# sreeramkannan/Shannon

Measured on AMD Instinct MI355X. Metric: reads/sec k-mer->graph->path-decompose, 2x100bp k=25, higher is better.
Workload: dtype u64

## Files before the change

shannon_amd/csrc/extend.hip:

```cpp
#include "common.h"
#include <cstring>
#include <vector>
#include <time.h>
#include <cstdio>
#include <cstdlib>
#include <algorithm>

#define EBLK 256
#define WBLK 64
#define UNCLAIMED 0xFFFFFFFFu
#define NONE32 0xFFFFFFFFu
#define UNCLAIMED64 0xFFFFFFFFFFFFFFFFULL
#define NOHINT_WORD 0xFFFFFFFFu
#define LONG_WALK 8
#define MEMO_MIN 1
#define PROMOTE_STEPS 16
typedef unsigned long long u64;
#define CLAIM(rank, pos) (((u64)(rank) << 32) | (u64)(uint32_t)(pos))
#define RANK(c) ((uint32_t)((c) >> 32))
#define POS(c) ((uint32_t)(c))

struct Adj4 { int32_t v[4]; };
struct __attribute__((aligned(64))) Rec {
  Adj4 R;
// ... 1171 lines not shown
  if (isd && lg) long_list[bl + ol + __popcll(lm & below)] = (uint32_t)r;
  if (isd && !lg) short_list[bs + os + __popcll(sm & below)] = (uint32_t)r;
}

__global__ void ext_memo_plan_kernel(uint8_t* __restrict__ ran, uint8_t* __restrict__ dirty,
                                     const uint32_t* __restrict__ nr, const uint32_t* __restrict__ nl, const uint32_t* __restrict__ order,
                                     uint32_t frozen, uint32_t limit, uint64_t* __restrict__ moff, uint32_t* __restrict__ mR,
                                     uint32_t* __restrict__ mL, uint8_t* __restrict__ mvalid, uint8_t* __restrict__ fill,
                                     uint32_t* __restrict__ pool, unsigned long long* __restrict__ cursor, uint64_t pool_cap, uint32_t memo_min,
                                     uint32_t* __restrict__ log_head = nullptr) {
  uint64_t r = (uint64_t)blockIdx.x * blockDim.x + threadIdx.x + frozen;
  if (r >= limit) return;
  const uint8_t did_run = dirty[r];
  ran[r] = did_run;
  dirty[r] = 0;
  if (log_head && did_run && memo_min != 0xFFFFFFFFu) log_head[r] = (nr[r] != UNCLAIMED && nr[r] + nl[r] == 0) ? NONE32 : LOG_LOST;
  uint8_t f = 0;
  if (did_run && nr[r] != UNCLAIMED) {
    const uint32_t R = nr[r], L = nl[r];
    if (R + L >= memo_min) {
      const uint64_t cap = (uint64_t)R + L + 5;
      const unsigned long long off = atomicAdd(cursor, (unsigned long long)cap);
      if (off + cap + 64 <= pool_cap) {
        pool[off] = MEMO_MARK; pool[off + 1] = R | MEMO_HI; pool[off + 2] = order[r];
        pool[off + 3 + R] = MEMO_MARK; pool[off + 4 + R + L] = MEMO_MARK;
        moff[r] = off; mR[r] = R; mL[r] = L; mvalid[r] = 2; f = 1;
      }
    }
  }
  if (did_run && !f && mvalid[r]) mvalid[r] = 1;
  fill[r] = f;
}

__global__ __launch_bounds__(64) void ext_release_memo_kernel(const uint32_t* __restrict__ long_list, uint64_t n_long, const uint32_t* __restrict__ short_list,
                                                              uint64_t n_short, const uint32_t* __restrict__ nr, const uint64_t* __restrict__ moff,
                                                              const uint32_t* __restrict__ mR, const uint32_t* __restrict__ mL, const uint32_t* __restrict__ pool,
                                                              u64* claim, uint8_t* __restrict__ chunk, const uint8_t* __restrict__ mvalid = nullptr,
                                                              const uint32_t* __restrict__ order = nullptr, const uint32_t* __restrict__ logpool = nullptr,
                                                              const uint32_t* __restrict__ log_head = nullptr, const uint8_t* __restrict__ log_cnt = nullptr) {
  const uint64_t idx = blockIdx.x;
  if (idx >= n_long + n_short) return;
  const uint32_t r = idx < n_long ? long_list[idx] : short_list[idx - n_long];
  if (nr[r] == UNCLAIMED) return;
  if (mvalid && mvalid[r] != 2) {
    auto give_back = [&](uint32_t node) {
      const u64 c = __hip_atomic_load(&claim[node], __ATOMIC_RELAXED, __HIP_MEMORY_SCOPE_AGENT);
      if (RANK(c) == r && atomicCAS(&claim[node], c, UNCLAIMED64) == c && chunk) chunk[node >> CHUNK_SHIFT] = 1;
    };
    if (threadIdx.x == 0) give_back(order[r]);
    uint32_t ch = log_head[r], cnt = log_cnt[r];
    while (ch != NONE32 && ch != LOG_LOST) {
      const uint32_t* c = logpool + (uint64_t)ch * LOG_WORDS;
      if (threadIdx.x >= 1 && threadIdx.x <= cnt) give_back(c[threadIdx.x]);
      ch = c[0];
      cnt = LOG_PER;
    }
    return;
  }
  const uint64_t off = moff[r];
  const uint32_t R = mR[r], L = mL[r];
  for (uint32_t j = threadIdx.x; j <= R + L; j += 64) {
    const uint32_t node = pool[off + (j <= R ? 2 : 3) + j];
    if (node & 0x80000000u) continue;
    if (atomicCAS(&claim[node], CLAIM(r, j), UNCLAIMED64) == CLAIM(r, j) && chunk) chunk[node >> CHUNK_SHIFT] = 1;
  }
}
// ... 82 lines not shown
#undef MARK
  };
  if (!chunk) {
    for (uint64_t ch = wave; ch < n_groups; ch += n_waves) {
      const uint64_t y = (ch << 6) + lane;
      uint32_t a;
      if (y < n2 && mark_node(y, a)) mark_around(y, a);
    }
  } else {
    static_assert(CHUNK_SHIFT == 4, "four line flags per group of 64 k1-mers");
    const uint64_t n_super = (n_groups + 63) >> 6;
    for (uint64_t sg = wave; sg < n_super; sg += n_waves) {
      const uint64_t g = (sg << 6) + lane;
      const uint32_t fl = g < n_groups ? *(const uint32_t*)(chunk + g * 4) : 0u;
      unsigned long long todo = __ballot(fl != 0);
      while (todo) {
        const int j = __ffsll((long long)todo) - 1;
        todo &= todo - 1;
        const uint32_t flj = (uint32_t)__shfl((int)fl, j, 64);
        const uint64_t y = ((((sg << 6) + (uint64_t)j)) << 6) + lane;
        uint32_t a = 0;
        if (y < n2 && ((flj >> (8 * (lane >> 4))) & 0xFFu) && mark_node(y, a)) mark_around(y, a);
      }
    }
  }
  __shared__ unsigned long long blk_changed;
  if (threadIdx.x == 0) blk_changed = 0;
  __syncthreads();
  if (my_changed) atomicAdd(&blk_changed, (unsigned long long)my_changed);
  __syncthreads();
  if (threadIdx.x == 0 && blk_changed) atomicAdd(n_changed, blk_changed);
}

__global__ void ext_verify_kernel(const uint8_t* __restrict__ ran, uint8_t* __restrict__ robbed, uint64_t ns, uint8_t* __restrict__ dirty) {
  uint64_t r = (uint64_t)blockIdx.x * blockDim.x + threadIdx.x;
  if (r >= ns) return;
  if (robbed[r]) { robbed[r] = 0; if (ran[r]) dirty[r] = 1; }
}

__global__ void ext_seed_rank_kernel(const uint32_t* __restrict__ order, uint64_t ns, Rec* __restrict__ rec) {
  uint64_t r = (uint64_t)blockIdx.x * blockDim.x + threadIdx.x;
  if (r < ns) rec[order[r]].seed_rank = (uint32_t)r;
}

__global__ void ext_select_kernel(const uint32_t* __restrict__ ranks, uint64_t n_sel, int32_t* __restrict__ sel_of_rank,
                                  unsigned long long* __restrict__ n_twice) {
  uint64_t t = (uint64_t)blockIdx.x * blockDim.x + threadIdx.x;
  if (t >= n_sel) return;
  if (atomicCAS((int*)&sel_of_rank[ranks[t]], -1, (int)t) != -1) atomicAdd(n_twice, 1ULL);
}

__global__ void ext_emit_claims_kernel(const u64* __restrict__ claim, uint64_t n2, const int32_t* __restrict__ sel_of_rank, uint64_t ns,
                                       const uint32_t* __restrict__ nr_a, const uint32_t* __restrict__ nl_a,
                                       const uint64_t* __restrict__ tkeys, int k, const uint64_t* __restrict__ out_off,
                                       uint8_t* __restrict__ out_bases, unsigned long long* __restrict__ counters) {
  uint32_t n_wrote = 0, n_stray = 0;
  for (uint64_t y = (uint64_t)blockIdx.x * blockDim.x + threadIdx.x; y < n2; y += (uint64_t)gridDim.x * blockDim.x) {
    const u64 c = claim[y];
    const uint32_t r = RANK(c), pos = POS(c);
    if (r == UNCLAIMED || r >= ns) continue;
    const int32_t t = sel_of_rank[r];
    if (t < 0) continue;
    const uint32_t nr = nr_a[r], nl = nl_a[r];
    if (nr == UNCLAIMED || pos > nr + nl) { n_stray++; continue; }
    uint8_t* dst = out_bases + out_off[t];
    const uint64_t str = oriented_string(tkeys, (uint32_t)y, k);
    if (pos == 0) for (int j = 0; j < k; j++) dst[nl + j] = "ACGT"[(str >> (2 * (k - 1 - j))) & 3];
    else if (pos <= nr) dst[nl + k + (pos - 1)] = "ACGT"[str & 3];
    else dst[nl - 1 - (pos - nr - 1)] = "ACGT"[(str >> (2 * (k - 1))) & 3];
    n_wrote++;
// ... 539 lines not shown
  if (!e->has_dig) return shn_fail(SHN_ERR_ARG, "shn_ext_digests: the extension was not made with SHN_EXT_DIGEST=1");
  memcpy(out, e->dig, sizeof e->dig);
  return SHN_OK;
}

extern "C" int shn_extend(shn_ctx* ctx, const shn_table* t, uint32_t min_weight, int max_iterations, shn_ext** out) {
  return shn_extend_sharded(ctx, t, min_weight, max_iterations, 1, 0, out);
}

extern "C" int shn_extend_sharded(shn_ctx* ctx, const shn_table* t, uint32_t min_weight, int max_iterations, int world, int rank,
                                  shn_ext** out) {
  if (!ctx || !t || !out) return shn_fail(SHN_ERR_ARG, "shn_extend: NULL argument");
  if (world < 1 || world > 255 || rank < 0 || rank >= world) return shn_fail(SHN_ERR_ARG, "shn_extend_sharded: bad world/rank");
  if (2 * t->n >= 0x7FFFFFFFULL) return shn_fail(SHN_ERR_ARG, "shn_extend: table too large for 31-bit oriented ids");
  SHN_ENTER(ctx);
  shn_stage_begin(ctx);
  hipStream_t s = ctx->stream; shn_use_stream(s);
  if (world > 1 && t->n) {
    shn_table* sub = nullptr;
    int rcs;
    { TimerRegion treg(ctx, T_EXTEND); rcs = component_shard(ctx, t, world, rank, &sub); }
    if (rcs) return rcs;
    rcs = shn_extend_sharded(ctx, sub, min_weight, max_iterations, 1, 0, out);
    if (rcs) { shn_table_destroy(sub); return rcs; }
    (*out)->owned_table = sub;
    return SHN_OK;
  }
  TimerRegion treg(ctx, T_EXTEND);
  shn_ext* e = new shn_ext();
  memset(e, 0, sizeof(*e));
  e->ctx = ctx; e->device = ctx->device; e->k = t->k; e->n = t->n; e->min_weight = min_weight; e->table = t;
  uint64_t n = t->n;
  if (max_iterations <= 0) max_iterations = 100000;
#define TRYE(x) do { hipError_t _e = (x); if (_e != hipSuccess) { shn_ext_destroy(e); \
      return shn_fail(SHN_ERR_HIP, std::string(#x) + ": " + hipGetErrorString(_e)); } } while (0)
  TRYE(shn_dev_malloc(&e->d_weight, (n + 1) * 4));
  TRYE(shn_dev_malloc(&e->d_flags, n + 1));
  TRYE(shn_dev_malloc(&e->d_rec, (2 * n + 1) * sizeof(Rec)));
  const uint64_t claim_words = (2 * n + 4 + 31) & ~31ULL;
  { u64* both = nullptr;
    TRYE(shn_dev_malloc(&both, std::max<uint64_t>(2 * claim_words * 8, fine_dict_lines(t) * 128)));
    e->d_claim = both; e->d_claim2 = both + claim_words; }
  if (n) {
    TimerRegion t1(ctx, T_EXT_PREP);
    hipLaunchKernelGGL(ext_prepare_kernel, dim3((uint32_t)cdiv(n, 256)), dim3(256), 0, s, t->d_keys, t->d_counts, n, t->k,
                       t->canonical, e->d_weight, e->d_flags);
    {
      unsigned long long* lines = nullptr;
      uint64_t n_lines = 0;
      { int rca = build_fine_dict(ctx, t, e->d_flags, &lines, &n_lines, e->d_claim); if (rca) { shn_ext_destroy(e); return rca; } }
      static const bool rec_lds = getenv("SHN_REC_LDS") && getenv("SHN_REC_LDS")[0] == '1';
      if (t->layout == 1 && rec_lds && t->n_buckets / REC_G + 1 < 0x7FFFFFFFULL) {
        TimerRegion ta(ctx, T_EXT_ADJ);
        hipLaunchKernelGGL(ext_records_lds_kernel, dim3((uint32_t)cdiv(t->n_buckets, REC_G)), dim3(256), 0, s, shn_tab_idx(t), e->d_flags, e->d_weight,
                           (uint64_t)t->n_buckets, t->k, t->canonical, e->d_rec, (const unsigned long long*)lines,
                           getenv("SHN_REC_ABLATE") ? atoi(getenv("SHN_REC_ABLATE")) : 0);
      } else
      { TimerRegion ta(ctx, T_EXT_ADJ);
        hipLaunchKernelGGL(ext_records_kernel, dim3((uint32_t)std::min<uint64_t>(cdiv(n * 8, 256), 1u << 22)), dim3(256), 0, s, shn_tab_idx(t),
                           e->d_flags, e->d_weight, n, t->k, t->canonical, e->d_rec, (const unsigned long long*)lines, n_lines,
                           (getenv("SHN_XCD_MAP") && getenv("SHN_XCD_MAP")[0] == '1') ? 1 : 0); }
      (void)lines;
    }
    TRYE(hipGetLastError());
  }
  void *pk, *pv, *pk2, *pv2, *pc;
  int rc;
  if ((rc = shn_ws(ctx)[13].get(2048, &pc))) { shn_ext_destroy(e); return rc; }
  unsigned long long* d_cnt = (unsigned long long*)pc;
  TRYE(hipMemsetAsync(d_cnt, 0, 2048, s));
  const uint64_t n_sblk = cdiv(n, 1024);
  uint32_t* d_bcnt = nullptr; uint64_t* d_bbase = nullptr;
  struct SeedScratch { uint32_t** a; uint64_t** b; ~SeedScratch() { if (*a) shn_dev_free(*a); if (*b) shn_dev_free(*b); } } seed_scratch{&d_bcnt, &d_bbase};
  TRYE(shn_dev_malloc(&d_bcnt, (n_sblk + 1) * 4));
  TRYE(shn_dev_malloc(&d_bbase, (n_sblk + 2) * 8));
  if (n) hipLaunchKernelGGL(ext_seed_kernel, dim3((uint32_t)n_sblk), dim3(1024), 0, s, t->d_keys, e->d_weight, e->d_flags, n,
                            t->k, t->canonical, min_weight, d_bcnt, (const uint64_t*)nullptr, (uint64_t*)nullptr, (uint32_t*)nullptr);
  uint64_t ns = 0;
  if (n && (rc = shn_device_scan_u32(ctx, d_bcnt, n_sblk, d_bbase, &ns))) { shn_ext_destroy(e); return rc; }
  if ((rc = shn_ws(ctx)[9].get((ns + 2) * 8, &pk)) || (rc = shn_ws(ctx)[10].get((ns + 2) * 4, &pv)) ||
      (rc = shn_ws(ctx)[11].get((ns + 2) * 8, &pk2)) || (rc = shn_ws(ctx)[12].get((ns + 2) * 4, &pv2))) { shn_ext_destroy(e); return rc; }
  uint64_t* skeys = (uint64_t*)pk; uint32_t* svals = (uint32_t*)pv;
  if (n) hipLaunchKernelGGL(ext_seed_kernel, dim3((uint32_t)n_sblk), dim3(1024), 0, s, t->d_keys, e->d_weight, e->d_flags, n,
                            t->k, t->canonical, min_weight, d_bcnt, (const uint64_t*)d_bbase, skeys, svals);
  e->n_seeds = ns;
  {
    TimerRegion t2(ctx, T_EXT_SORT);
    if ((rc = shn_sort_pairs(ctx, skeys, svals, (uint64_t*)pk2, (uint32_t*)pv2, ns, 0, 2 * t->k))) { shn_ext_destroy(e); return rc; }
    if (ns) {
      hipLaunchKernelGGL(ext_weightkey_kernel, dim3((uint32_t)cdiv(ns, 256)), dim3(256), 0, s, svals, e->d_weight, ns, skeys);
      if ((rc = shn_sort_pairs(ctx, skeys, svals, (uint64_t*)pk2, (uint32_t*)pv2, ns, 0, 32))) { shn_ext_destroy(e); return rc; }
    }
  }
  TRYE(shn_dev_malloc(&e->d_order, (ns + 1) * 4));
  TRYE(shn_dev_malloc(&e->d_nr, (ns + 1) * 4));
  TRYE(shn_dev_malloc(&e->d_nl, (ns + 1) * 4));
  TRYE(shn_dev_malloc(&e->d_totw, (ns + 1) * 8));
  uint64_t pool_cap = std::min<uint64_t>(24 * n + (1ULL << 20), (1ULL << 30) - 1);
  if (getenv("SHN_EXT_POOL_WORDS")) pool_cap = std::max<uint64_t>(256, std::min<uint64_t>(pool_cap, strtoull(getenv("SHN_EXT_POOL_WORDS"), nullptr, 10)));
  TRYE(hipMemcpyAsync(e->d_order, svals, ns * 4, hipMemcpyDeviceToDevice, s));
  TRYE(hipMemsetAsync(e->d_nr, 0xFF, (ns + 1) * 4, s));
  TRYE(hipMemsetAsync(e->d_nl, 0, (ns + 1) * 4, s));
  TRYE(hipMemsetAsync(e->d_totw, 0, (ns + 1) * 8, s));
  TRYE(hipMemsetAsync(e->d_claim, 0xFF, (2 * n + 4) * 8, s));
  void *ppool, *pplan;
  if ((rc = shn_ws(ctx)[27].get(pool_cap * 4, &ppool)) ||
      (rc = shn_ws(ctx)[28].get((ns + 1) * (8 + 4 * 10 + 1 + 1 + 1 + 1 + 1 + 1 + 1) + 64, &pplan))) { shn_ext_destroy(e); return rc; }
  u64 *claim = e->d_claim, *snap = e->d_claim2;
  uint32_t* pool = (uint32_t*)ppool;
  uint64_t* moff = (uint64_t*)pplan;
  uint32_t* mcap = (uint32_t*)(moff + ns + 1);
  uint32_t* mR = mcap + ns + 1;
  uint32_t* mL = mR + ns + 1;
  uint32_t* long_list = mL + ns + 1;
  uint32_t* short_list = long_list + ns + 1;
  uint32_t* promo_list = short_list + ns + 1;
  uint32_t* res_cur = promo_list + ns + 1;
  uint32_t* res_info = res_cur + ns + 1;
  uint32_t* owned = res_info + ns + 1;
  uint32_t* log_head = owned + ns + 1;
  uint8_t* mvalid = (uint8_t*)(log_head + ns + 1);
  uint8_t* fill = mvalid + ns + 1;
  uint8_t* dirty = fill + ns + 1;
  uint8_t* ran = dirty + ns + 1;
  uint8_t* robbed = ran + ns + 1;
  uint8_t* settled = robbed + ns + 1;
  uint8_t* log_cnt = settled + ns + 1;
  TRYE(hipMemsetAsync(robbed, 0, 2 * (ns + 1), s));
  TRYE(hipMemsetAsync(log_head, 0xFE, (ns + 1) * 4, s));
  uint8_t* robsat = nullptr;
  struct RobsatFree { uint8_t** p; ~RobsatFree() { if (*p) shn_dev_free(*p); } } robsat_free{&robsat};
  if (getenv("SHN_EXT_XTIME")) { TRYE(shn_dev_malloc(&robsat, ns + 1)); TRYE(hipMemsetAsync(robsat, 0, ns + 1, s)); }
  TRYE(hipMemsetAsync(mvalid, 0, 2 * (ns + 1), s));
  TRYE(hipMemsetAsync(pool, 0xFF, pool_cap * 4, s));
  if (ns) hipLaunchKernelGGL(ext_seed_rank_kernel, dim3((uint32_t)cdiv(ns, 256)), dim3(256), 0, s, e->d_order, (uint64_t)ns, e->d_rec);
  const bool want_dig = getenv("SHN_EXT_DIGEST") && getenv("SHN_EXT_DIGEST")[0] == '1';
  if (want_dig) {
    int rd;
    if ((rd = ext_digest(ctx, e, 0, t->d_keys, n * 8, 1)) || (rd = ext_digest(ctx, e, 1, t->d_counts, n * 4, 2)) ||
        (rd = ext_digest(ctx, e, 2, t->d_bucket_off, (t->n_buckets + 1) * 8, 3)) || (rd = ext_digest(ctx, e, 3, e->d_weight, n * 4, 4)) ||
        (rd = ext_digest(ctx, e, 3, e->d_flags, n & ~3ULL, 5)) || (rd = ext_digest(ctx, e, 4, e->d_rec, 2 * n * sizeof(Rec), 6)) ||
        (rd = ext_digest(ctx, e, 5, e->d_order, ns * 4, 7))) { shn_ext_destroy(e); return rd; }
  }
  hipStream_t aux = nullptr;
  hipEvent_t ev_fork = nullptr, ev_join = nullptr;
  TRYE(hipStreamCreateWithFlags(&aux, hipStreamNonBlocking));
  TRYE(hipEventCreateWithFlags(&ev_fork, hipEventDisableTiming));
  TRYE(hipEventCreateWithFlags(&ev_join, hipEventDisableTiming));
  static thread_local unsigned long long* plan = nullptr;
  if (!plan) TRYE(hipHostMalloc((void**)&plan, 64));
  int it = 0, repairs = 0;
  bool converged = ns == 0;
  uint8_t* chunk = nullptr;
  const uint64_t n_chunks = ((2 * n) >> CHUNK_SHIFT) + 16;
  TRYE(shn_dev_malloc(&chunk, n_chunks));
  struct ChunkFree { uint8_t* p; ~ChunkFree() { shn_dev_free(p); } } chunk_free{chunk};
  TRYE(hipMemsetAsync(chunk, 0, n_chunks, s));
  uint8_t* coarse = nullptr;
  TRYE(shn_dev_malloc(&coarse, (size_t)ns / 64 + 64));
  struct CoarseFree { uint8_t* p; ~CoarseFree() { shn_dev_free(p); } } coarse_free{coarse};
  bool snap_current = false;
  bool fresh_block = true;

  const uint32_t g2n = (uint32_t)cdiv(2 * n, 256);
  const bool many = ns >= (1ULL << 24);
  unsigned long long lim0 = std::max<unsigned long long>(ns / (many ? 8 : 32), 4096), grow = 4;
  if (getenv("SHN_EXT_LIMIT0")) lim0 = strtoull(getenv("SHN_EXT_LIMIT0"), nullptr, 10);
  if (getenv("SHN_EXT_GROW")) grow = strtoull(getenv("SHN_EXT_GROW"), nullptr, 10);
  const unsigned long long tail_div = getenv("SHN_EXT_TAIL") ? strtoull(getenv("SHN_EXT_TAIL"), nullptr, 10) : (many ? 0 : 8);
  uint32_t frozen = 0, limit = (uint32_t)std::min<unsigned long long>(ns, lim0);
  TRYE(hipMemsetAsync(dirty, 0, 2 * (ns + 1), s));
  TRYE(hipMemsetAsync(dirty, 1, limit, s));
  TRYE(hipMemsetAsync(owned, 0, (ns + 1) * 4, s));
  plan[6] = 64;
  TRYE(hipMemcpyAsync(d_cnt + 10, plan + 6, 8, hipMemcpyHostToDevice, s));
  auto tune = [](const char* name, uint32_t dflt) { const char* v = getenv(name); return v ? (uint32_t)strtoul(v, nullptr, 10) : dflt; };
  const int precise_marks = (int)tune("SHN_EXT_PRECISE", 1);
  const uint32_t long_walk = tune("SHN_EXT_LONG_WALK", LONG_WALK), memo_min = tune("SHN_EXT_MEMO_MIN", MEMO_MIN),
                 promote_steps = tune("SHN_EXT_PROMOTE", PROMOTE_STEPS);
  const unsigned long long bulk_min = getenv("SHN_EXT_BULK") ? strtoull(getenv("SHN_EXT_BULK"), nullptr, 10) : 262144ULL;
  const unsigned long long dense_min = getenv("SHN_EXT_DENSE") ? strtoull(getenv("SHN_EXT_DENSE"), nullptr, 10) : (4ULL << 20);
  const int seed_check = (int)tune("SHN_EXT_SEEDCHECK", 1);
  const int first_look = (int)tune("SHN_EXT_FIRST_LOOK", 0);
  const uint32_t bulk_promote = tune("SHN_EXT_PROMOTE_BULK", 0);
  const unsigned long long resume_waves = tune("SHN_EXT_RESUME_WAVES", 8192);
  const bool skip_idle_begin = tune("SHN_EXT_MEMO_RELEASE", 1) != 0;
  const unsigned long long memo_release_max = tune("SHN_EXT_MEMO_RELEASE_MAX", 65536);
  int n_begin_skipped = 0;
  const bool prepass = tune("SHN_EXT_PREPASS", 1) != 0;
  const uint32_t settle_hops = tune("SHN_EXT_SETTLE_HOPS", 0);
  const bool use_logs = tune("SHN_EXT_LOGS", 1) != 0 && bulk_promote == 0 && ns > 0;
  const unsigned long long targeted_max_steps = getenv("SHN_EXT_TARGETED_MAX") ? strtoull(getenv("SHN_EXT_TARGETED_MAX"), nullptr, 10) : (12ULL << 20);
  uint32_t* logpool = nullptr;
  struct LogFree { uint32_t** p; ~LogFree() { if (*p) shn_dev_free(*p); } } log_free{&logpool};
  uint64_t log_cap = use_logs ? std::min<uint64_t>(2 * n / 4 + (1u << 16), 0x7FFFFFF0ULL) : 0;
  if (use_logs && getenv("SHN_EXT_LOG_CHUNKS")) log_cap = std::max<uint64_t>(LOG_SLAB, std::min<uint64_t>(log_cap, strtoull(getenv("SHN_EXT_LOG_CHUNKS"), nullptr, 10)));
  if (use_logs) { TRYE(shn_dev_malloc(&logpool, log_cap * LOG_WORDS * 4)); TRYE(hipMemsetAsync(d_cnt + 26, 0, 8, s)); }
  const uint32_t fresh_split = std::max<uint32_t>(1, std::min<uint32_t>(16, tune("SHN_EXT_FRESH_SPLIT", 1)));
  const uint32_t fresh_split_min = tune("SHN_EXT_FRESH_SPLIT_MIN", 65536);
  unsigned long long expect_dirty = limit;
  while (!converged && it < max_iterations) {
    const bool bulk = bulk_min && expect_dirty >= bulk_min;
    const bool dense = bulk && expect_dirty >= dense_min;
    TRYE(hipMemsetAsync(d_cnt + 2, 0, 32, s));
    TRYE(hipMemsetAsync(d_cnt + 24, 0, 8, s));
    if (limit > frozen)
      hipLaunchKernelGGL(ext_plan_kernel, dim3((uint32_t)cdiv(limit - frozen, 1024)), dim3(1024), 0, s, e->d_nr, e->d_nl, (uint64_t)limit, frozen,
                         mvalid, mR, mL, dirty, long_list, short_list, d_cnt + 2, bulk ? 0xFFFFFFFFu : long_walk, coarse,
                         (fresh_block && frozen > 0 && prepass) ? (const u64*)claim : (const u64*)nullptr, e->d_order, e->d_totw,
                         (const Rec*)e->d_rec, fresh_block ? settle_hops : 0u, settled, d_cnt + 20, robsat, d_cnt + 21,
                         use_logs ? (const uint32_t*)log_head : (const uint32_t*)nullptr, d_cnt + 24);
    TRYE(hipMemcpyAsync(plan, d_cnt + 2, 32, hipMemcpyDeviceToHost, s));
    TRYE(hipMemcpyAsync(plan + 7, d_cnt + 24, 8, hipMemcpyDeviceToHost, s));
    TRYE(hipStreamSynchronize(s));
    expect_dirty = plan[3];
    if (plan[3] == 0) {
      if (limit >= ns) {
        TimerRegion ta(ctx, T_EXT_AUDIT);
        TRYE(hipMemsetAsync(owned, 0, (ns + 1) * 4, s));
        TRYE(hipMemsetAsync(d_cnt + 48, 0, 16, s));
        hipLaunchKernelGGL(ext_audit_nodes_kernel, dim3(std::min<uint32_t>(g2n, 4096u)), dim3(256), 0, s, claim, 2 * n, rows_R(e->d_rec),
                           rows_L(e->d_rec), words_weight(e->d_rec), e->d_order, e->d_nr, e->d_nl, (uint64_t)ns, owned, dirty, d_cnt + 48);
        hipLaunchKernelGGL(ext_audit_walks_kernel, dim3((uint32_t)cdiv(ns, 256)), dim3(256), 0, s, claim, e->d_order, e->d_nr, e->d_nl, (uint64_t)ns,
                           owned, dirty, d_cnt + 48);
        TRYE(hipMemcpyAsync(plan + 4, d_cnt + 48, 16, hipMemcpyDeviceToHost, s));
        TRYE(hipStreamSynchronize(s));
        if (plan[4] == 0 && plan[5] == 0) {
          converged = true;
          if (g_block_cb) g_block_cb(g_block_user, e, frozen, ns, 1);
          break;
        }
        if (g_block_cb) g_block_cb(g_block_user, e, 0, 0, -1);
        fprintf(stderr, "[shn_extend] fixpoint audit after %d rounds: %llu k1-mers / %llu walks disagree with the greedy rule; reopening all blocks\n",
                it, plan[4], plan[5]);
        if (++repairs > 16) break;
        fresh_block = false;
        frozen = 0;
        expect_dirty = plan[4] + plan[5];
        TRYE(hipMemsetAsync(ran, 0, ns + 1, s));
// ... 79 lines not shown
    if (plan[2]) {
      TimerRegion tk(ctx, fresh_block ? T_EXT_WALK_FRESH : T_EXT_WALK_THREAD);
      if (fresh_block) hipLaunchKernelGGL(ext_walk_kernel<true>, dim3((uint32_t)cdiv(plan[2], WBLK)), dim3(WBLK), 0, s, A, (uint64_t)plan[2], short_list, snap);
      else hipLaunchKernelGGL(ext_walk_kernel<false>, dim3((uint32_t)cdiv(plan[2], WBLK)), dim3(WBLK), 0, s, A, (uint64_t)plan[2], short_list, snap);
    }
    if (x_t0 > 0) {
      TRYE(hipStreamSynchronize(s)); timespec ts; clock_gettime(CLOCK_MONOTONIC, &ts);
      unsigned long long st = 0, lw = 0; TRYE(hipMemcpyAsync(&st, d_cnt + 1, 8, hipMemcpyDeviceToHost, s));
      if (A.dbg) { TRYE(hipMemcpyAsync(&lw, d_cnt + 44, 8, hipMemcpyDeviceToHost, s)); TRYE(hipMemsetAsync(d_cnt + 44, 0, 8, s)); }
      TRYE(hipStreamSynchronize(s));
      unsigned long long nrs[3] = {0, 0, 0}; TRYE(hipMemcpyAsync(nrs, d_cnt + 21, 24, hipMemcpyDeviceToHost, s)); TRYE(hipMemsetAsync(d_cnt + 21, 0, 24, s)); TRYE(hipStreamSynchronize(s));
      fprintf(stderr, "[shn_extend] XTIME round %d [%u,%u): of the claim holders without a memo %llu were robbed while they sat out; their walks: longest %llu steps, %llu steps in all\n", it + 1, frozen, limit, nrs[0], nrs[1], nrs[2]);
      fprintf(stderr, "[shn_extend] XTIME round %d: release %s (claims to give back by the records: %llu; bulk %d dense %d fresh %d snapshot current %d)\n", it + 1,
              was_fresh ? "none (a new block)" : memo_release_done ? "through memos / logs" : "the begin pass", plan[7], (int)bulk, (int)dense, (int)was_fresh, (int)snap_was_current);
      fprintf(stderr, "[shn_extend] XTIME round %d: %llu dirty walks, %llu of them hold claims without a current memo (rounds released through memos so far: %d); thread walker %llu walks, %.2f ms, steps so far %llu; longest walk %llu steps in %.2f ms (%.2f us per step)\n", it + 1, plan[3], plan[1], n_begin_skipped, plan[2],
              ts.tv_sec * 1e3 + ts.tv_nsec * 1e-6 - x_t0, st, lw >> 32, (double)(lw & 0xFFFFFFFFULL) * 1e-5, (lw >> 32) ? (double)(lw & 0xFFFFFFFFULL) * 1e-2 / (double)(lw >> 32) : 0.0);
    }
    if (plan[2] && bulk) {
      if (bulk_promote) {
        TimerRegion tk(ctx, T_EXT_WALK_THREAD);
        const uint32_t rgrid = (uint32_t)std::min<unsigned long long>(cdiv(plan[2], WBLK), resume_waves);
        if (was_fresh) hipLaunchKernelGGL(ext_walk_resume_kernel<true>, dim3(rgrid), dim3(WBLK), 0, s, A, promo_list, (const unsigned long long*)(d_cnt + 13), d_cnt + 14, snap);
        else hipLaunchKernelGGL(ext_walk_resume_kernel<false>, dim3(rgrid), dim3(WBLK), 0, s, A, promo_list, (const unsigned long long*)(d_cnt + 13), d_cnt + 14, snap);
      }
    } else if (plan[2]) {
      TimerRegion tk(ctx, T_EXT_WALK_WAVE);
      hipLaunchKernelGGL(ext_walk_long_kernel<true>, dim3((uint32_t)std::min<unsigned long long>(plan[2], 8192ULL)), dim3(64), 0, s, A, promo_list,
                         (uint64_t)ns, (const unsigned long long*)(d_cnt + 13));
    }
    if (plan[0]) TRYE(hipStreamWaitEvent(s, ev_join, 0));
    const bool skip_mark = fresh_block && bulk && precise_marks;
    fresh_block = false;
    if (dense) e->dense_rounds++;
    hipLaunchKernelGGL(ext_memo_plan_kernel, dim3((uint32_t)cdiv(limit - frozen, 256)), dim3(256), 0, s, ran, dirty, e->d_nr, e->d_nl, e->d_order, frozen, limit,
                       moff, mR, mL, mvalid, fill, pool, d_cnt + 10, pool_cap, bulk ? 0xFFFFFFFFu : memo_min, use_logs ? log_head : (uint32_t*)nullptr);
    if (skip_mark) { snap_current = false; if (!dense) TRYE(hipMemsetAsync(chunk, 0, n_chunks, s)); }
    else
    { TimerRegion tk(ctx, T_EXT_MARK);
      hipLaunchKernelGGL(ext_mark_kernel, dim3(std::min<uint32_t>(g2n, 4096u)), dim3(256), 0, s, claim, snap, 2 * n, e->d_rec,
                         dirty, ran, d_cnt + 6, frozen, limit, bulk ? (const uint8_t*)nullptr : (const uint8_t*)fill, moff, mR, pool, e->d_nr, e->d_nl, precise_marks,
                         dense ? (const uint8_t*)nullptr : chunk, robsat);
      if (!dense) TRYE(hipMemsetAsync(chunk, 0, n_chunks, s)); }
    hipLaunchKernelGGL(ext_verify_kernel, dim3((uint32_t)cdiv(ns, 256)), dim3(256), 0, s, ran, robbed, (uint64_t)ns, dirty);
    if (getenv("SHN_EXT_FAULT") && it + 1 == atoi(getenv("SHN_EXT_FAULT"))) TRYE(hipMemsetAsync(dirty, 0, ns + 1, s));
    if (getenv("SHN_EXT_ALLDIRTY")) { TRYE(hipMemsetAsync(dirty, 0, ns + 1, s)); TRYE(hipMemsetAsync(dirty + frozen, 1, limit - frozen, s)); }
    it++;

    if (getenv("SHN_DEBUG")) {
      unsigned long long chg = 0, cur = 0, mx[2] = {0, 0}, st_tr[2] = {0, 0};
      TRYE(hipMemcpyAsync(&st_tr[0], d_cnt + 1, 8, hipMemcpyDeviceToHost, s));
      TRYE(hipMemcpyAsync(&st_tr[1], d_cnt + 15, 8, hipMemcpyDeviceToHost, s));
      TRYE(hipMemcpyAsync(&chg, d_cnt + 6, 8, hipMemcpyDeviceToHost, s));
      TRYE(hipMemcpyAsync(&cur, d_cnt + 10, 8, hipMemcpyDeviceToHost, s));
      TRYE(hipMemcpyAsync(mx, d_cnt + 42, 16, hipMemcpyDeviceToHost, s));
      TRYE(hipMemsetAsync(d_cnt + 42, 0, 16, s));
      TRYE(hipStreamSynchronize(s));
      static double t_prev = 0;
      timespec ts; clock_gettime(CLOCK_MONOTONIC, &ts);
      double tn = ts.tv_sec * 1e3 + ts.tv_nsec * 1e-6;
      static unsigned long long st_prev[2] = {0, 0};
      if (it == 1) { st_prev[0] = st_prev[1] = 0; }
      fprintf(stderr, "[shn_extend] round %d [%u,%u): dirty=%llu long=%llu short=%llu changed_kmers=%llu pool=%.1f%% longest wavefront walk: %llu steps, most sequential: %llu (no hint %llu, owner without memo %llu, memo moved on %llu, followed %llu)  thread steps %llu in %llu wavefront trips (lanes busy %.3f)  %.2f ms\n", it, frozen, limit,
              plan[3], plan[0], plan[2], chg, 100.0 * (double)cur / (double)pool_cap, mx[1], mx[0] >> 48, (mx[0] >> 36) & 4095, (mx[0] >> 24) & 4095, (mx[0] >> 12) & 4095, mx[0] & 4095,
              st_tr[0] - st_prev[0], st_tr[1] - st_prev[1], (double)(st_tr[0] - st_prev[0]) / (64.0 * (double)std::max<unsigned long long>(1, st_tr[1] - st_prev[1])), it == 1 ? 0.0 : tn - t_prev);
      st_prev[0] = st_tr[0]; st_prev[1] = st_tr[1];
      t_prev = tn;
    }
  }
  hipStreamSynchronize(aux);
  hipStreamDestroy(aux);
  hipEventDestroy(ev_fork);
  hipEventDestroy(ev_join);
  if (converged && ns && getenv("SHN_EXT_AUDIT")) {
    WalkArgs A;
    memset(&A, 0, sizeof(A));
    A.order = e->d_order; A.adjR = rows_R(e->d_rec); A.adjL = rows_L(e->d_rec); A.weight = words_weight(e->d_rec);
    A.claim = claim; A.nr_out = e->d_nr; A.nl_out = e->d_nl; A.totw_out = e->d_totw;
    unsigned long long au[2] = {0, ~0ULL};
    plan[4] = 0; plan[5] = ~0ULL;
    TRYE(hipMemcpyAsync(d_cnt + 48, plan + 4, 16, hipMemcpyHostToDevice, s));
    hipLaunchKernelGGL(ext_audit_kernel, dim3((uint32_t)cdiv(ns, 64)), dim3(64), 0, s, A, (uint64_t)ns, d_cnt + 48);
    TRYE(hipMemcpyAsync(plan + 4, d_cnt + 48, 16, hipMemcpyDeviceToHost, s));
    TRYE(hipStreamSynchronize(s));
    au[0] = plan[4]; au[1] = plan[5];
    if (au[0]) {
      fprintf(stderr, "[shn_extend] AUDIT: %llu walks are not at their fixpoint, lowest rank %llu of %llu (rounds %d)\n", au[0], au[1], ns, it);
      if (atoi(getenv("SHN_EXT_AUDIT")) > 1) { shn_ext_destroy(e); return shn_fail(SHN_ERR_INTERNAL, "shn_extend: audit failed"); }
    }
  }
  e->iterations = it;
  if (!converged) { shn_ext_destroy(e); return shn_fail(SHN_ERR_INTERNAL, "shn_extend: walk fixpoint did not converge"); }
  if (want_dig) {
    int rd;
    if ((rd = ext_digest(ctx, e, 6, claim, 2 * n * 8, 8)) || (rd = ext_digest(ctx, e, 7, e->d_nr, ns * 4, 9)) || (rd = ext_digest(ctx, e, 7, e->d_nl, ns * 4, 10)) ||
        (rd = ext_digest(ctx, e, 7, e->d_totw, ns * 8, 11))) { shn_ext_destroy(e); return rd; }
  }
  TRYE(hipStreamSynchronize(s));
  shn_dev_free(e->d_rec); e->d_rec = nullptr;
  e->d_claim2 = nullptr;
  unsigned long long steps = 0, wsteps = 0, fsteps = 0, wslots[64];
  TRYE(hipMemcpyAsync(&steps, d_cnt + 1, 8, hipMemcpyDeviceToHost, s));
  TRYE(hipMemcpyAsync(&fsteps, d_cnt + 16, 8, hipMemcpyDeviceToHost, s));
  { unsigned long long nset = 0; TRYE(hipMemcpyAsync(&nset, d_cnt + 20, 8, hipMemcpyDeviceToHost, s)); TRYE(hipStreamSynchronize(s)); e->settled_walks = nset; }
  TRYE(hipMemcpyAsync(wslots, d_cnt + 64, 64 * 8, hipMemcpyDeviceToHost, s));
  TRYE(hipStreamSynchronize(s));
  for (int i = 0; i < 64; i++) wsteps += wslots[i];
  steps += wsteps;
  if (getenv("SHN_DEBUG")) {
    unsigned long long dbg[10];
    TRYE(hipMemcpyAsync(dbg, d_cnt + 32, 80, hipMemcpyDeviceToHost, s));
    TRYE(hipStreamSynchronize(s));
    fprintf(stderr, "[shn_extend] converged after %d rounds; steps: %llu total, %llu in the wave kernel (%llu from own memos, %llu from foreign memos)\n",
            it, steps, wsteps, dbg[0], dbg[1]);
    fprintf(stderr, "[shn_extend] memo_follow: no hint %llu, owner without memo %llu, memo moved on %llu, followed backwards %llu, nothing left %llu, followed %llu; "
            "chunks broken at the first step %llu, later %llu\n", dbg[2], dbg[3], dbg[4], dbg[5], dbg[6], dbg[7], dbg[8], dbg[9]);
  }
  e->total_steps = steps;
  e->wave_steps = wsteps;
  e->fresh_steps = fsteps;
  TRYE(hipGetLastError());
#undef TRYE
  *out = e;
  return SHN_OK;
}

extern "C" uint64_t shn_ext_n_walks(const shn_ext* e) { return e ? e->n_seeds : 0; }
extern "C" int shn_ext_iterations(const shn_ext* e) { return e ? e->iterations : 0; }
extern "C" uint64_t shn_ext_total_steps(const shn_ext* e) { return e ? e->total_steps : 0; }
// ... 267 lines not shown
```

Baseline: 67.84 million.

## Add sparse 16-flag-per-thread plan, memo-plan and verify kernels for sparse rounds

Adds planning and memo-planning kernels in which each thread loads 16 dirty flags as two 64-bit words and processes only the rows that are set. They are used when a round is expected to be sparse, meaning not a fresh block, no robsat, and fewer dirty rows than the range size. The verify kernel is rewritten the same way so it skips over clean robbed bytes. This cuts per-row memory traffic and thread count in late fixpoint rounds where few walks are dirty, but the sparse plan drops the claim/order prepass arguments and relies on the sparse kernel matching the dense one's counters and list order. The aux stream creation is moved earlier with cleanup lambdas so error paths release it.

```diff
diff --git a/shannon_amd/csrc/extend.hip b/shannon_amd/csrc/extend.hip
--- a/shannon_amd/csrc/extend.hip
+++ b/shannon_amd/csrc/extend.hip
@@ -1227,6 +1227,138 @@
   fill[r] = f;
 }
 
+struct W16 { unsigned long long lo, hi; };
+__device__ __forceinline__ W16 ld_flags16(const uint8_t* p, uint32_t n) {
+  W16 w;
+  if (n >= 16) { __builtin_memcpy(&w, p, 16); return w; }
+  w.lo = w.hi = 0;
+  for (uint32_t j = 0; j < n; j++) { const unsigned long long b = p[j]; if (j < 8) w.lo |= b << (8 * j); else w.hi |= b << (8 * (j - 8)); }
+  return w;
+}
+__device__ __forceinline__ void st_flags16(uint8_t* p, const W16 w, uint32_t n) {
+  if (n >= 16) { __builtin_memcpy(p, &w, 16); return; }
+  for (uint32_t j = 0; j < n; j++) p[j] = (uint8_t)((j < 8 ? w.lo >> (8 * j) : w.hi >> (8 * (j - 8))) & 0xFFu);
+}
+__device__ __forceinline__ uint32_t nonzero_bytes16(const W16 w) {
+  uint32_t m = 0;
+  if (w.lo | w.hi) {
+#pragma unroll
+    for (int j = 0; j < 8; j++) { m |= ((w.lo >> (8 * j)) & 0xFFu) ? 1u << j : 0u; m |= ((w.hi >> (8 * j)) & 0xFFu) ? 1u << (8 + j) : 0u; }
+  }
+  return m;
+}
+
+__global__ __launch_bounds__(256) void ext_plan_sparse_kernel(uint32_t* nr, uint32_t* nl, uint32_t limit, uint32_t frozen,
+                                const uint8_t* __restrict__ mvalid, const uint32_t* __restrict__ mR, const uint32_t* __restrict__ mL,
+                                const uint8_t* __restrict__ dirty, uint32_t* __restrict__ long_list, uint32_t* __restrict__ short_list,
+                                unsigned long long* __restrict__ counters, uint32_t long_walk, uint8_t* __restrict__ coarse,
+                                uint64_t* __restrict__ totw, const uint8_t* __restrict__ settled, const uint32_t* __restrict__ log_head,
+                                unsigned long long* __restrict__ rel_steps) {
+  const uint64_t t = (uint64_t)blockIdx.x * blockDim.x + threadIdx.x;
+  const uint64_t r0 = (uint64_t)frozen + 16 * t;
+  const int lane = threadIdx.x & 63, wid = threadIdx.x >> 6;
+  uint32_t m = 0;
+  if (r0 < limit) m = nonzero_bytes16(ld_flags16(dirty + r0, (uint32_t)std::min<uint64_t>(16, limit - r0)));
+  const unsigned long long anyd = __ballot(m != 0);
+  if ((lane & 3) == 0 && r0 < limit) coarse[t >> 2] = ((anyd >> lane) & 0xFULL) ? 1 : 0;
+  uint32_t live = 0, lg = 0;
+  uint32_t nd = 0, nh = 0;
+  unsigned long long st = 0;
+  for (uint32_t mm = m; mm; mm &= mm - 1) {
+    const uint32_t j = (uint32_t)__ffs(mm) - 1;
+    const uint64_t r = r0 + j;
+    nd++;
+    uint32_t a = nr[r];
+    const uint8_t mv = mvalid[r];
+    if (settled[r]) { nr[r] = UNCLAIMED; nl[r] = 0; totw[r] = 0; a = UNCLAIMED; }
+    else {
+      uint32_t len = a == UNCLAIMED ? 0 : a + nl[r];
+      if (mv) len = max(len, mR[r] + mL[r]);
+      live |= 1u << j;
+      if (len >= long_walk) lg |= 1u << j;
+    }
+    if (a != UNCLAIMED) {
+      const bool has_log = mv != 2 && log_head && log_head[r] != LOG_LOST;
+      if (mv != 2 && !has_log) nh++;
+      if (rel_steps) st += (unsigned long long)a + nl[r] + 1ULL;
+    }
+  }
+  const uint32_t mine = (uint32_t)__popc(lg) | ((uint32_t)__popc(live & ~lg) << 16);
+  uint32_t incl = mine;
+  __shared__ uint32_t wsum[4];
+  __shared__ unsigned long long bl, bs, acc[3];
+  if (threadIdx.x < 3) acc[threadIdx.x] = 0;
+  if (anyd) {
+    for (int o = 1; o < 64; o <<= 1) { const uint32_t v = __shfl_up(incl, o, 64); if (lane >= o) incl += v; }
+  }
+  if (lane == 63) wsum[wid] = incl;
+  __syncthreads();
+  if (anyd) {
+    unsigned long long cnt = (unsigned long long)nd | ((unsigned long long)nh << 32);
+    for (int o = 32; o > 0; o >>= 1) { cnt += __shfl_down(cnt, o, 64); st += __shfl_down(st, o, 64); }
+    if (lane == 0) {
+      atomicAdd(&acc[0], cnt & 0xFFFFFFFFULL);
+      if (cnt >> 32) atomicAdd(&acc[1], cnt >> 32);
+      if (st) atomicAdd(&acc[2], st);
+    }
+  }
+  if (threadIdx.x == 0) {
+    uint32_t tot = 0;
+    for (int w = 0; w < (int)(blockDim.x >> 6); w++) tot += wsum[w];
+    bl = (tot & 0xFFFFu) ? atomicAdd(&counters[0], (unsigned long long)(tot & 0xFFFFu)) : 0ULL;
+    bs = (tot >> 16) ? atomicAdd(&counters[2], (unsigned long long)(tot >> 16)) : 0ULL;
+  }
+  __syncthreads();
+  if (threadIdx.x == 0) {
+    if (acc[0]) atomicAdd(&counters[3], acc[0]);
+    if (acc[1]) atomicAdd(&counters[1], acc[1]);
+    if (acc[2]) atomicAdd(rel_steps, acc[2]);
+  }
+  if (!live) return;
+  uint32_t before = incl - mine;
+  for (int w = 0; w < wid; w++) before += wsum[w];
+  uint64_t ol = bl + (before & 0xFFFFu), os = bs + (before >> 16);
+  for (uint32_t mm = live; mm; mm &= mm - 1) {
+    const uint32_t j = (uint32_t)__ffs(mm) - 1;
+    if ((lg >> j) & 1u) long_list[ol++] = (uint32_t)(r0 + j);
+    else short_list[os++] = (uint32_t)(r0 + j);
+  }
+}
+
+__global__ __launch_bounds__(256) void ext_memo_plan_sparse_kernel(uint8_t* __restrict__ ran, uint8_t* __restrict__ dirty,
+                                     const uint32_t* __restrict__ nr, const uint32_t* __restrict__ nl, const uint32_t* __restrict__ order,
+                                     uint32_t frozen, uint32_t limit, uint64_t* __restrict__ moff, uint32_t* __restrict__ mR,
+                                     uint32_t* __restrict__ mL, uint8_t* __restrict__ mvalid, uint8_t* __restrict__ fill,
+                                     uint32_t* __restrict__ pool, unsigned long long* __restrict__ cursor, uint64_t pool_cap, uint32_t memo_min,
+                                     uint32_t* __restrict__ log_head) {
+  const uint64_t r0 = (uint64_t)frozen + 16 * ((uint64_t)blockIdx.x * blockDim.x + threadIdx.x);
+  if (r0 >= limit) return;
+  const uint32_t n = (uint32_t)std::min<uint64_t>(16, limit - r0);
+  const W16 did = ld_flags16(dirty + r0, n);
+  W16 f; f.lo = f.hi = 0;
+  st_flags16(ran + r0, did, n);
+  st_flags16(dirty + r0, f, n);
+  for (uint32_t mm = nonzero_bytes16(did); mm; mm &= mm - 1) {
+    const uint32_t j = (uint32_t)__ffs(mm) - 1;
+    const uint64_t r = r0 + j;
+    const uint32_t R = nr[r], L = nl[r];
+    if (log_head && memo_min != 0xFFFFFFFFu) log_head[r] = (R != UNCLAIMED && R + L == 0) ? NONE32 : LOG_LOST;
+    bool slot = false;
+    if (R != UNCLAIMED && R + L >= memo_min) {
+      const uint64_t cap = (uint64_t)R + L + 5;
+      const unsigned long long off = atomicAdd(cursor, (unsigned long long)cap);
+      if (off + cap + 64 <= pool_cap) {
+        pool[off] = MEMO_MARK; pool[off + 1] = R | MEMO_HI; pool[off + 2] = order[r];
+        pool[off + 3 + R] = MEMO_MARK; pool[off + 4 + R + L] = MEMO_MARK;
+        moff[r] = off; mR[r] = R; mL[r] = L; mvalid[r] = 2; slot = true;
+        if (j < 8) f.lo |= 1ULL << (8 * j); else f.hi |= 1ULL << (8 * (j - 8));
+      }
+    }
+    if (!slot && mvalid[r]) mvalid[r] = 1;
+  }
+  st_flags16(fill + r0, f, n);
+}
+
 __global__ __launch_bounds__(64) void ext_release_memo_kernel(const uint32_t* __restrict__ long_list, uint64_t n_long, const uint32_t* __restrict__ short_list,
                                                               uint64_t n_short, const uint32_t* __restrict__ nr, const uint64_t* __restrict__ moff,
                                                               const uint32_t* __restrict__ mR, const uint32_t* __restrict__ mL, const uint32_t* __restrict__ pool,
@@ -1375,10 +1507,15 @@
   if (threadIdx.x == 0 && blk_changed) atomicAdd(n_changed, blk_changed);
 }
 
-__global__ void ext_verify_kernel(const uint8_t* __restrict__ ran, uint8_t* __restrict__ robbed, uint64_t ns, uint8_t* __restrict__ dirty) {
-  uint64_t r = (uint64_t)blockIdx.x * blockDim.x + threadIdx.x;
-  if (r >= ns) return;
-  if (robbed[r]) { robbed[r] = 0; if (ran[r]) dirty[r] = 1; }
+__global__ __launch_bounds__(256) void ext_verify_kernel(const uint8_t* __restrict__ ran, uint8_t* __restrict__ robbed, uint64_t ns, uint8_t* __restrict__ dirty) {
+  const uint64_t r0 = 16 * ((uint64_t)blockIdx.x * blockDim.x + threadIdx.x);
+  if (r0 >= ns) return;
+  const uint32_t n = (uint32_t)std::min<uint64_t>(16, ns - r0);
+  uint32_t mm = nonzero_bytes16(ld_flags16(robbed + r0, n));
+  if (!mm) return;
+  W16 zero; zero.lo = zero.hi = 0;
+  st_flags16(robbed + r0, zero, n);
+  for (; mm; mm &= mm - 1) { const uint64_t r = r0 + (uint32_t)__ffs(mm) - 1; if (ran[r]) dirty[r] = 1; }
 }
 
 __global__ void ext_seed_rank_kernel(const uint32_t* __restrict__ order, uint64_t ns, Rec* __restrict__ rec) {
@@ -1984,8 +2121,19 @@
   e->ctx = ctx; e->device = ctx->device; e->k = t->k; e->n = t->n; e->min_weight = min_weight; e->table = t;
   uint64_t n = t->n;
   if (max_iterations <= 0) max_iterations = 100000;
-#define TRYE(x) do { hipError_t _e = (x); if (_e != hipSuccess) { shn_ext_destroy(e); \
+  hipStream_t aux = nullptr;
+  hipEvent_t ev_fork = nullptr, ev_join = nullptr;
+  auto drop_aux = [&]() {
+    if (aux) { (void)hipStreamSynchronize(aux); (void)hipStreamDestroy(aux); aux = nullptr; }
+    if (ev_fork) { (void)hipEventDestroy(ev_fork); ev_fork = nullptr; }
+    if (ev_join) { (void)hipEventDestroy(ev_join); ev_join = nullptr; }
+  };
+  auto destroy_e = [&]() { drop_aux(); shn_ext_destroy(e); };
+#define TRYE(x) do { hipError_t _e = (x); if (_e != hipSuccess) { destroy_e(); \
       return shn_fail(SHN_ERR_HIP, std::string(#x) + ": " + hipGetErrorString(_e)); } } while (0)
+  TRYE(hipStreamCreateWithFlags(&aux, hipStreamNonBlocking));
+  TRYE(hipEventCreateWithFlags(&ev_fork, hipEventDisableTiming));
+  TRYE(hipEventCreateWithFlags(&ev_join, hipEventDisableTiming));
   TRYE(shn_dev_malloc(&e->d_weight, (n + 1) * 4));
   TRYE(shn_dev_malloc(&e->d_flags, n + 1));
   TRYE(shn_dev_malloc(&e->d_rec, (2 * n + 1) * sizeof(Rec)));
@@ -2000,7 +2148,7 @@
     {
       unsigned long long* lines = nullptr;
       uint64_t n_lines = 0;
-      { int rca = build_fine_dict(ctx, t, e->d_flags, &lines, &n_lines, e->d_claim); if (rca) { shn_ext_destroy(e); return rca; } }
+      { int rca = build_fine_dict(ctx, t, e->d_flags, &lines, &n_lines, e->d_claim); if (rca) { destroy_e(); return rca; } }
       static const bool rec_lds = getenv("SHN_REC_LDS") && getenv("SHN_REC_LDS")[0] == '1';
       if (t->layout == 1 && rec_lds && t->n_buckets / REC_G + 1 < 0x7FFFFFFFULL) {
         TimerRegion ta(ctx, T_EXT_ADJ);
@@ -2018,7 +2166,7 @@
   }
   void *pk, *pv, *pk2, *pv2, *pc;
   int rc;
-  if ((rc = shn_ws(ctx)[13].get(2048, &pc))) { shn_ext_destroy(e); return rc; }
+  if ((rc = shn_ws(ctx)[13].get(2048, &pc))) { destroy_e(); return rc; }
   unsigned long long* d_cnt = (unsigned long long*)pc;
   TRYE(hipMemsetAsync(d_cnt, 0, 2048, s));
   const uint64_t n_sblk = cdiv(n, 1024);
@@ -2029,19 +2177,19 @@
   if (n) hipLaunchKernelGGL(ext_seed_kernel, dim3((uint32_t)n_sblk), dim3(1024), 0, s, t->d_keys, e->d_weight, e->d_flags, n,
                             t->k, t->canonical, min_weight, d_bcnt, (const uint64_t*)nullptr, (uint64_t*)nullptr, (uint32_t*)nullptr);
   uint64_t ns = 0;
-  if (n && (rc = shn_device_scan_u32(ctx, d_bcnt, n_sblk, d_bbase, &ns))) { shn_ext_destroy(e); return rc; }
+  if (n && (rc = shn_device_scan_u32(ctx, d_bcnt, n_sblk, d_bbase, &ns))) { destroy_e(); return rc; }
   if ((rc = shn_ws(ctx)[9].get((ns + 2) * 8, &pk)) || (rc = shn_ws(ctx)[10].get((ns + 2) * 4, &pv)) ||
-      (rc = shn_ws(ctx)[11].get((ns + 2) * 8, &pk2)) || (rc = shn_ws(ctx)[12].get((ns + 2) * 4, &pv2))) { shn_ext_destroy(e); return rc; }
+      (rc = shn_ws(ctx)[11].get((ns + 2) * 8, &pk2)) || (rc = shn_ws(ctx)[12].get((ns + 2) * 4, &pv2))) { destroy_e(); return rc; }
   uint64_t* skeys = (uint64_t*)pk; uint32_t* svals = (uint32_t*)pv;
   if (n) hipLaunchKernelGGL(ext_seed_kernel, dim3((uint32_t)n_sblk), dim3(1024), 0, s, t->d_keys, e->d_weight, e->d_flags, n,
                             t->k, t->canonical, min_weight, d_bcnt, (const uint64_t*)d_bbase, skeys, svals);
   e->n_seeds = ns;
   {
     TimerRegion t2(ctx, T_EXT_SORT);
-    if ((rc = shn_sort_pairs(ctx, skeys, svals, (uint64_t*)pk2, (uint32_t*)pv2, ns, 0, 2 * t->k))) { shn_ext_destroy(e); return rc; }
+    if ((rc = shn_sort_pairs(ctx, skeys, svals, (uint64_t*)pk2, (uint32_t*)pv2, ns, 0, 2 * t->k))) { destroy_e(); return rc; }
     if (ns) {
       hipLaunchKernelGGL(ext_weightkey_kernel, dim3((uint32_t)cdiv(ns, 256)), dim3(256), 0, s, svals, e->d_weight, ns, skeys);
-      if ((rc = shn_sort_pairs(ctx, skeys, svals, (uint64_t*)pk2, (uint32_t*)pv2, ns, 0, 32))) { shn_ext_destroy(e); return rc; }
+      if ((rc = shn_sort_pairs(ctx, skeys, svals, (uint64_t*)pk2, (uint32_t*)pv2, ns, 0, 32))) { destroy_e(); return rc; }
     }
   }
   TRYE(shn_dev_malloc(&e->d_order, (ns + 1) * 4));
@@ -2057,7 +2205,7 @@
   TRYE(hipMemsetAsync(e->d_claim, 0xFF, (2 * n + 4) * 8, s));
   void *ppool, *pplan;
   if ((rc = shn_ws(ctx)[27].get(pool_cap * 4, &ppool)) ||
-      (rc = shn_ws(ctx)[28].get((ns + 1) * (8 + 4 * 10 + 1 + 1 + 1 + 1 + 1 + 1 + 1) + 64, &pplan))) { shn_ext_destroy(e); return rc; }
+      (rc = shn_ws(ctx)[28].get((ns + 1) * (8 + 4 * 10 + 1 + 1 + 1 + 1 + 1 + 1 + 1) + 64, &pplan))) { destroy_e(); return rc; }
   u64 *claim = e->d_claim, *snap = e->d_claim2;
   uint32_t* pool = (uint32_t*)ppool;
   uint64_t* moff = (uint64_t*)pplan;
@@ -2092,13 +2240,8 @@
     if ((rd = ext_digest(ctx, e, 0, t->d_keys, n * 8, 1)) || (rd = ext_digest(ctx, e, 1, t->d_counts, n * 4, 2)) ||
         (rd = ext_digest(ctx, e, 2, t->d_bucket_off, (t->n_buckets + 1) * 8, 3)) || (rd = ext_digest(ctx, e, 3, e->d_weight, n * 4, 4)) ||
         (rd = ext_digest(ctx, e, 3, e->d_flags, n & ~3ULL, 5)) || (rd = ext_digest(ctx, e, 4, e->d_rec, 2 * n * sizeof(Rec), 6)) ||
-        (rd = ext_digest(ctx, e, 5, e->d_order, ns * 4, 7))) { shn_ext_destroy(e); return rd; }
-  }
-  hipStream_t aux = nullptr;
-  hipEvent_t ev_fork = nullptr, ev_join = nullptr;
-  TRYE(hipStreamCreateWithFlags(&aux, hipStreamNonBlocking));
-  TRYE(hipEventCreateWithFlags(&ev_fork, hipEventDisableTiming));
-  TRYE(hipEventCreateWithFlags(&ev_join, hipEventDisableTiming));
+        (rd = ext_digest(ctx, e, 5, e->d_order, ns * 4, 7))) { destroy_e(); return rd; }
+  }
   static thread_local unsigned long long* plan = nullptr;
   if (!plan) TRYE(hipHostMalloc((void**)&plan, 64));
   int it = 0, repairs = 0;
@@ -2156,7 +2299,13 @@
     const bool dense = bulk && expect_dirty >= dense_min;
     TRYE(hipMemsetAsync(d_cnt + 2, 0, 32, s));
     TRYE(hipMemsetAsync(d_cnt + 24, 0, 8, s));
-    if (limit > frozen)
+    const bool whole_block = fresh_block || robsat != nullptr || expect_dirty >= (unsigned long long)(limit - frozen);
+    if (limit > frozen && !whole_block)
+      hipLaunchKernelGGL(ext_plan_sparse_kernel, dim3((uint32_t)cdiv(cdiv(limit - frozen, 16), 256)), dim3(256), 0, s, e->d_nr, e->d_nl, limit, frozen,
+                         (const uint8_t*)mvalid, (const uint32_t*)mR, (const uint32_t*)mL, (const uint8_t*)dirty, long_list, short_list, d_cnt + 2,
+                         bulk ? 0xFFFFFFFFu : long_walk, coarse, e->d_totw, (const uint8_t*)settled,
+                         use_logs ? (const uint32_t*)log_head : (const uint32_t*)nullptr, d_cnt + 24);
+    else if (limit > frozen)
       hipLaunchKernelGGL(ext_plan_kernel, dim3((uint32_t)cdiv(limit - frozen, 1024)), dim3(1024), 0, s, e->d_nr, e->d_nl, (uint64_t)limit, frozen,
                          mvalid, mR, mL, dirty, long_list, short_list, d_cnt + 2, bulk ? 0xFFFFFFFFu : long_walk, coarse,
                          (fresh_block && frozen > 0 && prepass) ? (const u64*)claim : (const u64*)nullptr, e->d_order, e->d_totw,
@@ -2302,8 +2451,13 @@
     const bool skip_mark = fresh_block && bulk && precise_marks;
     fresh_block = false;
     if (dense) e->dense_rounds++;
-    hipLaunchKernelGGL(ext_memo_plan_kernel, dim3((uint32_t)cdiv(limit - frozen, 256)), dim3(256), 0, s, ran, dirty, e->d_nr, e->d_nl, e->d_order, frozen, limit,
-                       moff, mR, mL, mvalid, fill, pool, d_cnt + 10, pool_cap, bulk ? 0xFFFFFFFFu : memo_min, use_logs ? log_head : (uint32_t*)nullptr);
+    if (whole_block)
+      hipLaunchKernelGGL(ext_memo_plan_kernel, dim3((uint32_t)cdiv(limit - frozen, 256)), dim3(256), 0, s, ran, dirty, e->d_nr, e->d_nl, e->d_order, frozen, limit,
+                         moff, mR, mL, mvalid, fill, pool, d_cnt + 10, pool_cap, bulk ? 0xFFFFFFFFu : memo_min, use_logs ? log_head : (uint32_t*)nullptr);
+    else
+      hipLaunchKernelGGL(ext_memo_plan_sparse_kernel, dim3((uint32_t)cdiv(cdiv(limit - frozen, 16), 256)), dim3(256), 0, s, ran, dirty, (const uint32_t*)e->d_nr,
+                         (const uint32_t*)e->d_nl, (const uint32_t*)e->d_order, frozen, limit, moff, mR, mL, mvalid, fill, pool, d_cnt + 10, pool_cap,
+                         bulk ? 0xFFFFFFFFu : memo_min, use_logs ? log_head : (uint32_t*)nullptr);
     if (skip_mark) { snap_current = false; if (!dense) TRYE(hipMemsetAsync(chunk, 0, n_chunks, s)); }
     else
     { TimerRegion tk(ctx, T_EXT_MARK);
@@ -2311,7 +2465,7 @@
                          dirty, ran, d_cnt + 6, frozen, limit, bulk ? (const uint8_t*)nullptr : (const uint8_t*)fill, moff, mR, pool, e->d_nr, e->d_nl, precise_marks,
                          dense ? (const uint8_t*)nullptr : chunk, robsat);
       if (!dense) TRYE(hipMemsetAsync(chunk, 0, n_chunks, s)); }
-    hipLaunchKernelGGL(ext_verify_kernel, dim3((uint32_t)cdiv(ns, 256)), dim3(256), 0, s, ran, robbed, (uint64_t)ns, dirty);
+    hipLaunchKernelGGL(ext_verify_kernel, dim3((uint32_t)cdiv(cdiv(ns, 16), 256)), dim3(256), 0, s, ran, robbed, (uint64_t)ns, dirty);
     if (getenv("SHN_EXT_FAULT") && it + 1 == atoi(getenv("SHN_EXT_FAULT"))) TRYE(hipMemsetAsync(dirty, 0, ns + 1, s));
     if (getenv("SHN_EXT_ALLDIRTY")) { TRYE(hipMemsetAsync(dirty, 0, ns + 1, s)); TRYE(hipMemsetAsync(dirty + frozen, 1, limit - frozen, s)); }
     it++;
@@ -2337,10 +2491,7 @@
       t_prev = tn;
     }
   }
-  hipStreamSynchronize(aux);
-  hipStreamDestroy(aux);
-  hipEventDestroy(ev_fork);
-  hipEventDestroy(ev_join);
+  drop_aux();
   if (converged && ns && getenv("SHN_EXT_AUDIT")) {
     WalkArgs A;
     memset(&A, 0, sizeof(A));
@@ -2355,15 +2506,15 @@
     au[0] = plan[4]; au[1] = plan[5];
     if (au[0]) {
       fprintf(stderr, "[shn_extend] AUDIT: %llu walks are not at their fixpoint, lowest rank %llu of %llu (rounds %d)\n", au[0], au[1], ns, it);
-      if (atoi(getenv("SHN_EXT_AUDIT")) > 1) { shn_ext_destroy(e); return shn_fail(SHN_ERR_INTERNAL, "shn_extend: audit failed"); }
+      if (atoi(getenv("SHN_EXT_AUDIT")) > 1) { destroy_e(); return shn_fail(SHN_ERR_INTERNAL, "shn_extend: audit failed"); }
     }
   }
   e->iterations = it;
-  if (!converged) { shn_ext_destroy(e); return shn_fail(SHN_ERR_INTERNAL, "shn_extend: walk fixpoint did not converge"); }
+  if (!converged) { destroy_e(); return shn_fail(SHN_ERR_INTERNAL, "shn_extend: walk fixpoint did not converge"); }
   if (want_dig) {
     int rd;
     if ((rd = ext_digest(ctx, e, 6, claim, 2 * n * 8, 8)) || (rd = ext_digest(ctx, e, 7, e->d_nr, ns * 4, 9)) || (rd = ext_digest(ctx, e, 7, e->d_nl, ns * 4, 10)) ||
-        (rd = ext_digest(ctx, e, 7, e->d_totw, ns * 8, 11))) { shn_ext_destroy(e); return rd; }
+        (rd = ext_digest(ctx, e, 7, e->d_totw, ns * 8, 11))) { destroy_e(); return rd; }
   }
   TRYE(hipStreamSynchronize(s));
   shn_dev_free(e->d_rec); e->d_rec = nullptr;
```

New measurement: 65.06 million. 0.959x the previous value.
